# dvl-tum/e-osvos

Measured on AMD Instinct MI355X. Metric: finetune_iters_per_sec, higher is better.
Workload: dtype f32 (f16x3 split); 1 GPU; e-OSVOS-50 fine-tune iteration (BASELINE configs[1]): DeepLabV3+-ResNet50, batch 3, 480x854, BCE, per-neuron-lr SGD; one (sequence, object) per rank; batch=3, height=480, width=854, parallelism=replicas x1

## Files before the change

e-osvos_amd/_ffi.py:

```python
import ctypes
import os

_HERE = os.path.dirname(os.path.abspath(__file__))
LIB_PATH = os.environ.get('EOSVOS_LIB') or os.path.join(_HERE, 'libeosvos.so')

c_float_p = ctypes.c_void_p
_E = ctypes.c_void_p


class View(ctypes.Structure):
    _fields_ = [('p', ctypes.c_void_p), ('ld', ctypes.c_int), ('key', ctypes.c_void_p), ('ldkey', ctypes.c_int)]


class ConvViews(ctypes.Structure):
    _fields_ = ([(n, ctypes.c_int) for n in ('algo', 'B', 'H', 'W', 'Cin', 'Cout', 'k', 'stride', 'dil', 'pad')] +
                [('w_oihw', ctypes.c_void_p), ('scale', ctypes.c_void_p), ('bias', ctypes.c_void_p), ('passes', ctypes.c_int),
                 ('x', View), ('y', View), ('res', View), ('relu', ctypes.c_int), ('y_m8', ctypes.c_void_p),
                 ('g', View), ('gx', View), ('add', View), ('accum', ctypes.c_int), ('mask_c0', ctypes.c_int),
                 ('gx_m8', ctypes.c_void_p), ('dw_oihw', ctypes.c_void_p),
                 ('slot_bits', ctypes.c_uint * 2), ('slot_valid', ctypes.c_int * 2),
                 ('src_slot_bits', ctypes.c_uint * 2), ('src_slot_valid', ctypes.c_int * 2), ('fwd_slices', ctypes.c_int)])


VIEWS_FWD, VIEWS_DGRAD, VIEWS_WGRAD = 1, 2, 4

_SIGNATURES = {
    'eosvos_version': (ctypes.c_char_p, []),
    'eosvos_last_error': (ctypes.c_char_p, []),
    'eosvos_set_matrix_mode': (ctypes.c_int, [ctypes.c_int]),
    'eosvos_get_matrix_mode': (ctypes.c_int, []),
    'eosvos_set_presplit': (ctypes.c_int, [ctypes.c_int]),
    'eosvos_plan_fingerprint': (ctypes.c_int, [_E, ctypes.POINTER(ctypes.c_uint64)]),
    'eosvos_set_engine_matrix_mode': (ctypes.c_int, [_E, ctypes.c_int]),
    'eosvos_get_engine_matrix_mode': (ctypes.c_int, [_E]),
    'eosvos_set_wg_budget': (ctypes.c_int, [_E, ctypes.c_int]),
    'eosvos_set_side_stream': (ctypes.c_int, [_E, ctypes.c_int]),
    'eosvos_num_convs': (ctypes.c_int, [ctypes.c_int]),
    'eosvos_conv_info': (ctypes.c_int, [ctypes.c_int, ctypes.c_int, ctypes.POINTER(ctypes.c_int64)]),
    'eosvos_param_count': (ctypes.c_int64, [ctypes.c_int]),
    'eosvos_lr_count': (ctypes.c_int64, [ctypes.c_int]),
    'eosvos_norm_count': (ctypes.c_int64, [ctypes.c_int]),
    'eosvos_create': (ctypes.c_int, [ctypes.POINTER(_E), ctypes.c_int, ctypes.c_int, ctypes.c_int,
                                     ctypes.c_int, ctypes.c_int, ctypes.c_int, ctypes.c_void_p]),
    'eosvos_create_ex': (ctypes.c_int, [ctypes.POINTER(_E), ctypes.c_int, ctypes.c_int, ctypes.c_int,
                                        ctypes.c_int, ctypes.c_int, ctypes.c_int, ctypes.c_void_p, ctypes.c_int]),
    'eosvos_destroy': (ctypes.c_int, [_E]),
# ... 190 lines not shown
```

e-osvos_amd/csrc/conv_kernels.hip:

```cpp
#include "kernels.h"
#include "conv_tile.h"

#include <stdlib.h>
#include <string.h>

#include <type_traits>
#include <vector>

namespace eosvos {

typedef float f32x16 __attribute__((ext_vector_type(16)));

#define EOSVOS_BK 32
#define EOSVOS_EB 4
#define EOSVOS_EB128 EOSVOS_EB
#define EOSVOS_OCC 2
#define MFMA32(a, b, c) __builtin_amdgcn_mfma_f32_32x32x2f32((a), (b), (c), 0, 0, 0)

#define EOSVOS_BK_DEEP 16
#define EOSVOS_DEEP_TILES 1024
template <int BN, bool KMAJOR, int DEEP = 0>
__global__ __launch_bounds__(256, DEEP ? 3 : EOSVOS_OCC) void conv_igemm_kernel(const ConvArgs p) {
  constexpr int BM = 128, BK = DEEP == 2 ? EOSVOS_BK_DEEP : EOSVOS_BK;
  constexpr int LDA = BK + 4;
// ... 1491 lines not shown
    const int ranges = a.N / NC;
    int chunks = (target + a.nplanes * ranges - 1) / (a.nplanes * ranges);
    const int max_chunks = a.plane_rows / 128 > 0 ? a.plane_rows / 128 : 1;
    chunks = chunks < 1 ? 1 : (chunks > max_chunks ? max_chunks : chunks);
    a.row_chunks = chunks;
    const int groups8 = (a.nplanes * chunks + 7) / 8 * 8;
    hipLaunchKernelGGL((conv1x1_stream_kernel<K, NC>), dim3(groups8 * ranges), dim3(512), lds, s, a);
    return;
  }
  constexpr int total = 256 * (K <= 128 ? EOSVOS_STREAM_OCC : 1);
  const int ranges = a.N / NC;
  const int wgs = total / ranges > 0 ? total / ranges : 1;
  hipLaunchKernelGGL((conv1x1_stream_kernel<K, NC>), dim3(wgs, ranges), dim3(512), lds, s, a);
}


#define STEM_SLOTS 24
#define STEM_PITCH (STEM_SLOTS * 16 + 32)
__global__ __launch_bounds__(512) void stem_fwd_h3_kernel(const float* __restrict__ xpad, const float* __restrict__ w,
                                                          const float* __restrict__ a, const float* __restrict__ bb,
                                                          float* __restrict__ y, int B, int H, int W, int Ho, int Wo,
                                                          const unsigned* __restrict__ amax_x) {
  __shared__ __attribute__((aligned(16))) unsigned char sw_[2 * 64 * STEM_PITCH];
  __shared__ float s_a[64], s_b[64];
  __shared__ unsigned s_red[8];
  const int tid = threadIdx.x, lane = tid & 63, wave = tid >> 6;
  float wv[3][8];
  unsigned wm = 0;
#pragma unroll
  for (int q = 0; q < 3; ++q) {
// ... 739 lines not shown
  }
  const int T = a.KH * a.KW;
  const int bk = a.deep == 2 ? EOSVOS_BK_DEEP : EOSVOS_BK;
  const long ksteps = (long)T * ((a.Kc + bk - 1) / bk);
  const long sk_tiles = tiles - (long)a.dp_q * nwg;
  const bool fixup = a.splitk > 1 || (a.per > 0 && sk_tiles > 0 && (a.per % ksteps != 0 || a.tprefix));
  if (g_plan_log_on)
    plan_log_add(ConvPlanRec{pk, a.kmajor != 0, bn, (int)tiles, (int)ksteps, a.deep, a.dp_q, a.per, nwg, a.splitk, a.tprefix != nullptr,
                             a.torder != nullptr, fixup, conv_wg_budget(a.wg_budget)});
  if (fixup) {
    ProfScope ps(kProfFixup, 0.0, s);
    with_tile(bn, [&](auto BN) { hipLaunchKernelGGL((conv_fixup_kernel<BN()>), dim3((unsigned)sk_tiles, 8), block, 0, s, a); });
  }
}

#define EOSVOS_WG_BKP 32
#define EOSVOS_WG_OCC 2
template <int BMO, int BNI>
__global__ __launch_bounds__(256, EOSVOS_WG_OCC) void wgrad_kernel(const WgradArgs p) {
  constexpr int BKP = EOSVOS_WG_BKP;
  constexpr int LDA = BMO + 4, LDB = BNI + 4;
  constexpr int A_EL = BKP * LDA, B_EL = BKP * LDB, STAGE = A_EL + B_EL;
  __shared__ __attribute__((aligned(16))) float smem[2 * STAGE];

  const int tid = threadIdx.x, lane = tid & 63, wave = tid >> 6;
  const int wm = wave >> 1, wn = wave & 1;
  const int r = lane & 31, h = lane >> 5;

  const int T = p.KH * p.KW;
  const int ct = (p.Cout + BMO - 1) / BMO, it = (p.Cin + BNI - 1) / BNI;
// ... 227 lines not shown
```

e-osvos_amd/csrc/engine.cpp:

```cpp
#include <dlfcn.h>
#include <hip/hip_runtime.h>
#include <math.h>
#include <stdio.h>
#include <stdlib.h>
#include <string.h>

#include <algorithm>
#include <cmath>
#include <functional>
#include <map>
#include <string>
#include <vector>

#include "../../include/eosvos.h"
#include "kernels.h"
#include "scratch_layout.h"
#include "tensor_views.h"

using namespace eosvos;

static thread_local std::string g_err;
static int fail(const std::string& m) {
  g_err = m;
  return 1;
// ... 633 lines not shown
  return m;
}
void wino_ensure_weights(eosvos_engine* e, int ci, int tm, hipStream_t st) {
  auto& w = e->wino[ci];
  if (w.us_valid) return;
  const ConvL& c = e->t.convs[ci];
  unsigned* us = amax_wino_weights(e, ci, st);
  launch_wino_weight(tm, e->W_(ci), c.cout, c.cin, e->A_(ci), w.U, w.Us, st, us, us ? us + e->t.convs.size() : nullptr);
  w.us_valid = true;
}
struct Opt {
  View add_;
  bool relu_ = false, side_ = false, accum_ = false;
  const Tensor* mask_ = nullptr;
  int mask_c0_ = 0;
  Opt& add(const View& v) { add_ = v; return *this; }
  Opt& relu(bool on = true) { relu_ = on; return *this; }
  Opt& side(bool on = true) { side_ = on; return *this; }
  Opt& accum(bool on = true) { accum_ = on; return *this; }
  Opt& mask(const Tensor* x, int c0 = 0) { mask_ = x; mask_c0_ = c0; return *this; }
};
void conv_fwd(eosvos_engine* e, int ci, const View& xv, const View& yv, int B, const Opt& o = Opt()) {
  const float *x = xv.ptr(), *res = o.add_.ptr();
  float* y = yv.ptr();
  const int ldx = xv.ld(), ldy = yv.ld(), ldres = o.add_.ld(), Hi = xv.t->H, Wi = xv.t->W;
  const bool relu = o.relu_, side = o.side_;
  const ConvL& c = e->t.convs[ci];
  ConvArgs a;
  memset(&a, 0, sizeof(a));
  a.wg_budget = e->wg_budget;
  hipStream_t st = side ? e->s2 : e->s;
  const Written yw = twrite_fused(e, yv);
  a.x = x; a.w = e->W_(ci); a.y = y; a.ws = side ? e->ws_conv2 : e->ws_conv;
  a.B = B; a.Hi = Hi; a.Wi = Wi; a.ldx = ldx; a.Kc = c.cin;
  a.Ho = conv_out(Hi, c.k, c.stride, c.dil, c.pad); a.Wo = conv_out(Wi, c.k, c.stride, c.dil, c.pad);
// ... 28 lines not shown
  } else {
    a.scale = e->A_(ci); a.bias = e->B_(ci);
    a.res = res; a.ldres = ldres; a.relu = relu ? 1 : 0;
    if (relu && yw.mask) { a.mask8_out = yw.mask; a.ldm8_out = yw.ldmask; }
  }
  attach_tap_table(e, ci, 0, B, a);
  if (h3_mode() && !amax_init(e)) {
    amax_weights(e, st);
    a.amax_x = tlookup(e, *xv.t);
    if (!a.amax_x) a.amax_x = amax_get(e, AM_X, ci, x, (long)B * Hi * Wi, c.cin, ldx, st);
    a.amax_w = amax_slot(e, AM_W, ci);
    if (!gn) a.amax_y = yw.slot;
  }
  if (!gn && !side) pair_attach(e, yv, a);
  trace("fwd", ci, a.M, a.N, (long)c.T() * c.cin, conv_plan(a), conv_exec_frac(a));
  launch_conv(a, st);
  pair_covered(e, *yv.t, a);
  if (gn)
    launch_gn_forward(e->zbuf[ci]->p, c.cout, e->G_(ci), e->nb + c.noff, res, ldres, y, ldy, e->gn_stats[ci], e->gn_partial, B,
                      a.Ho * a.Wo, c.cout, 1e-5f, relu ? 1 : 0, st, yw.slot, relu ? yw.mask : nullptr, yw.ldmask);
}
bool dgrad_has_tail(const ConvArgs& a) { return a.N > 128 && a.N % 128 > 0 && a.N % 128 <= 64; }
void launch_dgrad_tail_split(eosvos_engine* e, int ci, ConvArgs a, long K) {
  const int tail = a.N % 128;
  ConvArgs b = a;
  a.N -= tail;
  trace("dgrad", ci, a.M, a.N, K, conv_plan(a));
  launch_conv(a, e->s);
  b.N = tail; b.w += a.N; b.y += a.N;
  if (b.mask8) { b.mask8 += a.N / 4; b.mask_c0 = b.mask_c0 > a.N ? b.mask_c0 - a.N : 0; }
// ... 56 lines not shown
    launch_wino_dgrad_output(wg.tm, e->wino_dv, prow, c.cin, B, Hin, Win, th, tw, wg.d, mask8, a.ldm8, a.mask_c0, a.accum, gx, ldgx, e->s, gxs);
    return 0;
  }
  if (c.k == 1 && c.stride == 2 && !add) {
    if (!a.accum) (void)hipMemsetAsync(gx, 0, (size_t)B * Hin * Win * ldgx * sizeof(float), e->s);
    a.Ho = a.Hi; a.Wo = a.Wi; a.mul = 1; a.off0 = 0; a.kstep = 0; a.upshift = 0;
    a.M = B * a.Ho * a.Wo; a.dst_up = 1; a.Hf = Hin; a.Wf = Win;
  }
  if (dgrad_has_tail(a) && !a.dst_up && !(c.k == 3 && c.dil >= 2)) {
    launch_dgrad_tail_split(e, ci, a, (long)c.T() * c.cout);
    return 0;
  }
  attach_tap_table(e, ci, 1, B, a);
  pair_attach(e, gxv, a);
  trace("dgrad", ci, a.M, a.N, (long)c.T() * c.cout, conv_plan(a), conv_exec_frac(a));
  launch_conv(a, e->s);
  pair_covered(e, *gxv.t, a);
  return 0;
}
#define EOSVOS_SIDE_BATCH 4
int wgp_budget(const eosvos_engine* e) {
  constexpr int share = 75;
  int b = conv_wg_budget_of(e->wg_budget);
  if (e->s2) b = conv_clamp_wg_budget(std::max(64, b * share / 100 / 64 * 64));
  return b;
}
int pair_margin(int phase) {
  static const int margin_x = getenv("EOSVOS_TUNE_PAIR_MARGIN_X") ? atoi(getenv("EOSVOS_TUNE_PAIR_MARGIN_X")) : 2;
  static const int margin_g = getenv("EOSVOS_TUNE_PAIR_MARGIN_G") ? atoi(getenv("EOSVOS_TUNE_PAIR_MARGIN_G")) : 3;
  return phase == 0 ? margin_x : margin_g;
}
bool pair_operand(eosvos_engine* e, const View& v, long rows, PairBuf*& pb) {
  const long rows_alloc = e->lastB > 0 ? rows / e->lastB * e->maxB : rows;
// ... 431 lines not shown
  if (mode != EOSVOS_MATRIX_F32 && mode != EOSVOS_MATRIX_BF16X6 && mode != EOSVOS_MATRIX_F16X3) return fail("unknown matrix mode");
  conv_set_mfma_mode(mode);
  return 0;
}
int eosvos_get_matrix_mode(void) { return conv_mfma_mode(); }
int eosvos_plan_fingerprint(eosvos_engine* e, uint64_t* out2) {
  if (!e || !out2) return fail("null argument");
  out2[0] = e->plan_fp[0]; out2[1] = e->plan_fp[1];
  return 0;
}
int eosvos_set_presplit(int on) {
  const int prev = presplit_switch() ? g_presplit : 0;
  g_presplit = on == 2 ? 2 : (on ? 1 : 0);
  return prev;
}
int eosvos_set_engine_matrix_mode(eosvos_engine* e, int mode) {
  if (!e) return fail("null engine");
  if (mode != -1 && mode != EOSVOS_MATRIX_F32 && mode != EOSVOS_MATRIX_BF16X6 && mode != EOSVOS_MATRIX_F16X3) return fail("unknown matrix mode");
  e->mode = mode;
  return 0;
}
int eosvos_get_engine_matrix_mode(eosvos_engine* e) {
  if (!e) { fail("null engine"); return -1; }
  return e->mode >= 0 ? e->mode : conv_mfma_mode();
}
int eosvos_set_wg_budget(eosvos_engine* e, int workgroups) {
  if (!e) { fail("null engine"); return -1; }
  if (workgroups < 0) { fail("workgroup budget must be >= 0"); return -1; }
  const int b = conv_clamp_wg_budget(workgroups);
  if (b == e->wg_budget) return b;
// ... 534 lines not shown
    bool any = false;
    for (int ci = 0; ci < (int)e->wino.size(); ++ci) {
      if (!e->wino[ci].V || e->wino[ci].us_valid || ci >= (int)e->conv_hin.size() || !e->conv_hin[ci]) continue;
      const ConvL& c = t.convs[ci];
      const int Ho = conv_out(e->conv_hin[ci], c.k, c.stride, c.dil, c.pad), Wo = conv_out(e->conv_win[ci], c.k, c.stride, c.dil, c.pad);
      if (!wino_on(e, ci, B, Ho, Wo)) continue;
      if (!any) { fork(0); any = true; }
      wino_ensure_weights(e, ci, wino_geom(e, c, B, Ho, Wo).tm, e->s2);
    }
    if (any) { (void)hipEventRecord(e->ev_wino_w, e->s2); e->wino_w_wait = true; }
  }
  const View dcat_low(e->dcat, 256, 48);
  for (size_t i = 0; i < t.blocks.size(); ++i) {
    const Block& b = t.blocks[i];
    auto& f = e->bb[i];
    if (b.ds >= 0) {
      if (fside) fork(b.ds);
      conv_fwd(e, b.ds, f.xin, f.dsb, B, Opt().side(fside));
      if (fside) (void)hipEventRecord(e->ev[b.c3], e->s2);
    }
    conv_fwd(e, b.c1, f.xin, f.t1, B, Opt().relu());
    conv_fwd(e, b.c2, f.t1, f.t2, B, Opt().relu());
    if (b.ds >= 0 && fside) (void)hipStreamWaitEvent(s, e->ev[b.c3], 0);
    conv_fwd(e, b.c3, f.t2, f.out, B, Opt().relu().add(b.ds >= 0 ? f.dsb : f.xin));
    if ((int)i == t.layer1_last_block && fside && !t.v3) {
      fork(t.dec1);
      conv_fwd(e, t.dec1, f.out, dcat_low, B, Opt().relu().side());
      (void)hipEventRecord(e->ev[t.dec_a], e->s2);
    }
  }
  Tensor* const l4 = e->bb.back().out;
  const int P16 = e->h16 * e->w16;
  hipStream_t ps = fside ? e->s2 : s;
  if (fside) fork(t.pool);
  auto pool_branch = [&]() {
    launch_colsum(l4->p, l4->C, e->vec, B, P16, 2048, 1.0f / (float)P16, e->colscratch, ps);
    if (e->gn()) {
      launch_gemv_fwd(e->W_(t.pool), e->vec, nullptr, nullptr, e->zbuf[t.pool]->p, B, 256, 2048, ps);
      launch_gn_forward(e->zbuf[t.pool]->p, 256, e->G_(t.pool), e->nb + t.convs[t.pool].noff, nullptr, 0, e->poolout, 256,
// ... 126 lines not shown
  for (int i = l4_frozen ? -1 : (int)t.blocks.size() - 1; i >= 0; --i) {
    if (i == first_l4_block - 1) {
      if (flush_part0()) return 1;
      if (frozen) break;
    }
    const Block& b = t.blocks[i];
    auto& f = e->bb[i];
    conv_wgrad(e, b.c3, f.g_out, f.t2, B);
    if (conv_dgrad(e, b.c3, f.g_out, f.g_t2, B, Opt().mask(f.t2))) return 1;
    conv_wgrad(e, b.c2, f.g_t2, f.t1, B);
    if (conv_dgrad(e, b.c2, f.g_t2, f.g_t1, B, Opt().mask(f.t1))) return 1;
    const bool is_first_block = i == 0;
    bool have = !t.v3 && (i == t.layer1_last_block + 1);
    const Tensor* inmask = is_first_block ? nullptr : f.xin;
    const bool in_frozen = frozen && b.c1 == e->train_from;
    if (b.ds >= 0) {
      conv_wgrad(e, b.ds, f.g_out, f.xin, B);
      if (!in_frozen && conv_dgrad(e, b.ds, f.g_out, f.g_xin, B, Opt().accum(have))) return 1;
      conv_wgrad(e, b.c1, f.g_t1, f.xin, B);
      if (!in_frozen && conv_dgrad(e, b.c1, f.g_t1, f.g_xin, B, Opt().accum().mask(inmask))) return 1;
    } else {
      if (have) return fail("internal: identity block after the low-level tap is unsupported");
      conv_wgrad(e, b.c1, f.g_t1, f.xin, B);
      if (conv_dgrad(e, b.c1, f.g_t1, f.g_xin, B, Opt().mask(inmask).add(f.g_out))) return 1;
    }
    if (b.ds >= 0 && flush_wgrad_group(e, t.stage[b.c1], B)) return 1;
  }
  if (!frozen) {
  const auto& xrec = amax_rec_of(e, AM_X, 0);
  const bool stem_h3 = h3_mode() && e->amax && xrec.epoch == e->fwd_epoch && xrec.ptr == e->xpad;
  unsigned* ag = stem_h3 ? amax_fused_slot(e, AM_G, 0, e->gn() ? e->zbuf[0]->p : e->g_c1->p, s) : nullptr;
// ... 1966 lines not shown
```

e-osvos_amd/csrc/kernels.h:

```cpp
#pragma once
#include <hip/hip_runtime.h>
#include <stdint.h>

namespace eosvos {
#define AMAX_SUB 32
#define AMAX_ROW 2048
#if defined(__HIPCC__)
__device__ __forceinline__ unsigned amax_f1(float x) {
  const unsigned a = __float_as_uint(x) & 0x7fffffffu;
  return a < 0x7f800000u ? a : 0u;
}
__device__ __forceinline__ unsigned amax_f4(unsigned m, const float4& v) {
  const unsigned a = amax_f1(v.x), b = amax_f1(v.y), c = amax_f1(v.z), d = amax_f1(v.w);
  const unsigned ab = a > b ? a : b, cd = c > d ? c : d;
  const unsigned q = ab > cd ? ab : cd;
  return m > q ? m : q;
}
__device__ __forceinline__ uint8_t relu_bits(const float4& v) {
  return (uint8_t)((v.x > 0.f ? 1 : 0) | (v.y > 0.f ? 2 : 0) | (v.z > 0.f ? 4 : 0) | (v.w > 0.f ? 8 : 0));
}
__device__ __forceinline__ void relu_mask8(float4& v, unsigned bits) {
  v.x = (bits & 1u) ? v.x : 0.f; v.y = (bits & 2u) ? v.y : 0.f; v.z = (bits & 4u) ? v.z : 0.f; v.w = (bits & 8u) ? v.w : 0.f;
}
template <int WAVES = 4>
// ... 114 lines not shown
#endif
inline int conv_par_pixel(int B, int Ho, int Wo, int m) {
  const int He = (Ho + 1) >> 1, Hod = Ho >> 1, We = (Wo + 1) >> 1, Wod = Wo >> 1;
  const int n00 = B * He * We, n01 = B * He * Wod, n10 = B * Hod * We;
  int py, px, r = m;
  if (r < n00) { py = 0; px = 0; }
  else if ((r -= n00) < n01) { py = 0; px = 1; }
  else if ((r -= n01) < n10) { py = 1; px = 0; }
  else { r -= n10; py = 1; px = 1; }
  const int Hc = py ? Hod : He, Wc = px ? Wod : We;
  const int nc = Hc * Wc;
  const int b = r / nc, rr = r - b * nc;
  const int cy = rr / Wc, cx = rr - cy * Wc;
  return (b * Ho + 2 * cy + py) * Wo + 2 * cx + px;
}
void launch_conv(ConvArgs& a, hipStream_t s);
int conv_bn(const ConvArgs& a);
int conv_plan(ConvArgs& a);
void conv_set_mfma_mode(int mode);
void conv_set_thread_mfma_mode(int mode);
int conv_thread_mfma_mode();
void conv_prof_enable(int on);
int conv_prof_read(int max, const char** names, long* counts, double* ms, double* flops);
void conv_prof_mark_begin(int kernel, double flops, hipStream_t s);
void conv_prof_mark_end(hipStream_t s);
struct ConvPlanRec {
  int kernel;
  int kmajor, bn;
  int tiles, ksteps;
  int deep, dp_q, per, nwg, splitk;
  int tprefix, torder;
// ... 13 lines not shown
  X(kProfConvIgemm_2, "conv_igemm_kernel<64, false, 0>") X(kProfConvIgemm_3, "conv_igemm_kernel<64, true, 0>") \
  X(kProfWgrad, "wgrad_kernel<128, 128>") X(kProfWgrad_1, "wgrad_kernel<128, 64>") \
  X(kProfWgrad_2, "wgrad_kernel<64, 128>") X(kProfWgrad_3, "wgrad_kernel<64, 64>") \
  X(kProfFixup, "conv_fixup_kernel") \
  X(kProfWgradX6Group, "wgrad_x6_group_kernel<128, 128>") X(kProfWgradX6Group_1, "wgrad_x6_group_kernel<128, 64>") \
  X(kProfWgradX6Group_2, "wgrad_x6_group_kernel<64, 128>") X(kProfWgradX6Group_3, "wgrad_x6_group_kernel<64, 64>") \
  X(kProfConvH3, "conv_h3_kernel<128, false>") X(kProfConvH3_1, "conv_h3_kernel<128, true>") \
  X(kProfConvH3_2, "conv_h3_kernel<64, false>") X(kProfConvH3_3, "conv_h3_kernel<64, true>") \
  X(kProfWgradH3, "wgrad_h3_kernel<128, 128>") X(kProfWgradH3_1, "wgrad_h3_kernel<128, 64>") \
  X(kProfWgradH3_2, "wgrad_h3_kernel<64, 128>") X(kProfWgradH3_3, "wgrad_h3_kernel<64, 64>") \
  X(kProfWgradH3Group, "wgrad_h3_group_kernel<128, 128>") X(kProfWgradH3Group_1, "wgrad_h3_group_kernel<128, 64>") \
  X(kProfWgradH3Group_2, "wgrad_h3_group_kernel<64, 128>") X(kProfWgradH3Group_3, "wgrad_h3_group_kernel<64, 64>") \
  X(kProfConvH3Multi, "conv_h3_multi_kernel") X(kProfConvX6Multi, "conv_x6_multi_kernel") \
  X(kProfStream1x1_128, "conv1x1_stream_kernel<*, 128>") X(kProfStream1x1_64, "conv1x1_stream_kernel<*, 64>") \
  X(kProfStream3x3, "conv3x3_stream_kernel") \
  X(kProfWgradP, "wgrad_p_kernel<256, 256>") X(kProfWgradPGroup, "wgrad_p_group_kernel<256, 256>")
enum ProfKernel {
#define EOSVOS_PROF_ID(id, name) id,
  EOSVOS_PROF_KERNELS(EOSVOS_PROF_ID)
#undef EOSVOS_PROF_ID
  kProfKernels
};
double conv_exec_frac(const struct ConvArgs& a);
double wgrad_exec_frac(const struct WgradArgs& a);
int conv_mfma_mode();
void launch_absmax(const float* x, long rows, int C, int ld, unsigned* slot, hipStream_t s);
void launch_amax_zero(unsigned* first, int count, hipStream_t s);
void launch_absmax_segments(const float* base, const long* dev_off, const int* dev_n, int nseg, unsigned* slots, hipStream_t s);
double launch_mfma_probe(float* scratch, int iters, hipStream_t s);
int64_t conv_ws_floats();
}
// ... 295 lines not shown
```

e-osvos_amd/engine.py:

```python
import collections
import ctypes
import functools

import torch

from . import _ffi, bootstrap, boundary, cldice, loss_sum, potts, surface
from .loss_names import LOSS_KINDS, resolve_cap, resolve_loss, resolve_radius
from .topology import ARCH_ID, norm_layers, trainable


def _ptr(t):
    return ctypes.c_void_p(t.data_ptr())


def _optr(t):
    return _ptr(t) if t is not None else None


def _chunks(n, step):
    return ((f, min(f + step, n)) for f in range(0, n, step))


def _keep_flags(keep, n):
    flags = bytearray(n)
# ... 279 lines not shown
    def _check_images(self, images):
        self._check_stream()
        assert images.is_cuda and images.dtype == torch.float32 and images.is_contiguous()
        b, c, h, w = images.shape
        assert c == 3 and h == self.height and w == self.width and 1 <= b <= self.max_batch, images.shape
        return b

    @property
    def matrix_mode(self):
        return _MODE_NAMES[self.lib.eosvos_get_engine_matrix_mode(self.h)]

    def set_engine_matrix_mode(self, mode):
        _ffi.check(self.lib.eosvos_set_engine_matrix_mode(self.h, -1 if mode is None else _MODE_IDS[mode]))
        self._own_mode = mode
        self._guard_fell_back = False

    def plan_fingerprint(self):
        out = (ctypes.c_uint64 * 2)()
        _ffi.check(self.lib.eosvos_plan_fingerprint(self.h, out))
        return int(out[0]), int(out[1])

    def _new_state_for_guard(self):
        if getattr(self, '_guard_fell_back', False):
            self._guard_fell_back = False
            self.set_engine_matrix_mode(None)
        self._verify_pending = True

    def _fall_back(self, reason, diff, scale):
        import warnings
        self.set_engine_matrix_mode('bf16x6')
# ... 1044 lines not shown
```

include/eosvos.h:

```cpp
#ifndef EOSVOS_H
#define EOSVOS_H

#include <stddef.h>
#include <stdint.h>

#ifdef __cplusplus
extern "C" {
#endif

typedef struct eosvos_engine eosvos_engine;

#define EOSVOS_ARCH_RESNET50 50
#define EOSVOS_ARCH_RESNET101 101
#define EOSVOS_ARCH_V3_RESNET50 1050
#define EOSVOS_ARCH_V3_RESNET101 1101
#define EOSVOS_NORM_BN_FROZEN 0
#define EOSVOS_NORM_GN16 1

const char* eosvos_version(void);
const char* eosvos_last_error(void);

#define EOSVOS_MATRIX_F32 0
#define EOSVOS_MATRIX_BF16X6 1
#define EOSVOS_MATRIX_F16X3 2
int eosvos_set_matrix_mode(int mode);
int eosvos_get_matrix_mode(void);
int eosvos_set_presplit(int on);
int eosvos_plan_fingerprint(eosvos_engine* e, uint64_t* out2);
int eosvos_set_engine_matrix_mode(eosvos_engine* e, int mode);
int eosvos_get_engine_matrix_mode(eosvos_engine* e);

int eosvos_set_wg_budget(eosvos_engine* e, int workgroups);

int eosvos_set_side_stream(eosvos_engine* e, int on);

int eosvos_num_convs(int arch);
int eosvos_conv_info(int arch, int idx, int64_t* info);
int64_t eosvos_param_count(int arch);
int64_t eosvos_lr_count(int arch);
int64_t eosvos_norm_count(int arch);

int eosvos_create(eosvos_engine** out, int arch, int norm_mode, int height, int width,
// ... 266 lines not shown
```

Measured before the change: 114.9 finetune_iters/s.

## Fuse bottleneck main and downsample 1x1 convs into one branch-sum kernel

Adds a conv1x1_branch_kernel that computes the bottleneck's last 1x1 conv and its stride-1 downsample 1x1 conv in one launch and sums them in registers. In forward it replaces the side-stream downsample plus the residual-add conv. In backward it replaces the two dgrad launches that accumulate into the same input gradient. The aim is to drop a launch, a round trip of the downsample/intermediate tensor through memory, and a cross-stream event wait. The cost is that it only handles specific K/N shapes in f16x3 mode and gives up the side-stream overlap, and it falls back to the separate convs when the eligibility checks fail.

```diff
diff --git a/e-osvos_amd/_ffi.py b/e-osvos_amd/_ffi.py
--- a/e-osvos_amd/_ffi.py
+++ b/e-osvos_amd/_ffi.py
@@ -30,6 +30,8 @@
     'eosvos_set_matrix_mode': (ctypes.c_int, [ctypes.c_int]),
     'eosvos_get_matrix_mode': (ctypes.c_int, []),
     'eosvos_set_presplit': (ctypes.c_int, [ctypes.c_int]),
+    'eosvos_set_branch_fusion': (ctypes.c_int, [ctypes.c_int]),
+    'eosvos_test_branch_rowmap': (ctypes.c_int, [ctypes.c_int] * 4),
     'eosvos_plan_fingerprint': (ctypes.c_int, [_E, ctypes.POINTER(ctypes.c_uint64)]),
     'eosvos_set_engine_matrix_mode': (ctypes.c_int, [_E, ctypes.c_int]),
     'eosvos_get_engine_matrix_mode': (ctypes.c_int, [_E]),
diff --git a/e-osvos_amd/csrc/conv_kernels.hip b/e-osvos_amd/csrc/conv_kernels.hip
--- a/e-osvos_amd/csrc/conv_kernels.hip
+++ b/e-osvos_amd/csrc/conv_kernels.hip
@@ -1529,6 +1529,207 @@
   hipLaunchKernelGGL((conv1x1_stream_kernel<K, NC>), dim3(wgs, ranges), dim3(512), lds, s, a);
 }
 
+constexpr int br_it(int K, int NC) { return (NC * (K / 8) + 511) / 512; }
+template <int K, int NC, bool KMAJ>
+__device__ __forceinline__ void br_load_w(float (&raw)[br_it(K, NC)][8], const float* __restrict__ w, int wK, int n0, int tid) {
+  constexpr int GR = NC * (K / 8), IT = br_it(K, NC);
+#pragma unroll
+  for (int it = 0; it < IT; ++it) {
+    const int i = tid + it * 512;
+    if (!KMAJ) {
+      const int r = (i < GR ? i : 0) / (K / 8), c8 = i % (K / 8);
+      const float* src = w + (size_t)(n0 + r) * wK + c8 * 8;
+      const float4 lo = ldg4(src), hi = ldg4(src + 4);
+      raw[it][0] = lo.x; raw[it][1] = lo.y; raw[it][2] = lo.z; raw[it][3] = lo.w;
+      raw[it][4] = hi.x; raw[it][5] = hi.y; raw[it][6] = hi.z; raw[it][7] = hi.w;
+    } else {
+      const int c8 = (i < GR ? i : 0) / NC, r = i % NC;
+      const float* src = w + (size_t)(c8 * 8) * wK + n0 + r;
+#pragma unroll
+      for (int j = 0; j < 8; ++j) raw[it][j] = src[(size_t)j * wK];
+    }
+  }
+}
+template <int K, int NC, bool KMAJ>
+__device__ __forceinline__ void br_store_w(const float (&raw)[br_it(K, NC)][8], unsigned char* img, float sw, int tid) {
+  constexpr int GR = NC * (K / 8), IT = br_it(K, NC), PITCH = frag_pitch(K * 2);
+#pragma unroll
+  for (int it = 0; it < IT; ++it) {
+    const int i = tid + it * 512;
+    if (i < GR) {
+      const int r = KMAJ ? i % NC : i / (K / 8), c8 = KMAJ ? i / NC : i % (K / 8);
+      uint4 h0, h1;
+      s1_split8(make_float4(raw[it][0], raw[it][1], raw[it][2], raw[it][3]), make_float4(raw[it][4], raw[it][5], raw[it][6], raw[it][7]), sw, h0, h1);
+      *reinterpret_cast<uint4*>(img + r * PITCH + c8 * 16) = h0;
+      *reinterpret_cast<uint4*>(img + NC * PITCH + r * PITCH + c8 * 16) = h1;
+    }
+  }
+}
+template <int K, int NC, bool TILED>
+__device__ __forceinline__ void br_ksteps(float4 (&xr)[(K + 31) / 32][2], const float* qn, bool more, const float* s_ks, bool kscale, float sx,
+                                          const unsigned char* img, int fr, int fq, f32x4 (&acc)[NC / 16]) {
+  constexpr int KS = (K + 31) / 32, NF = NC / 16, FH = NF < 4 ? NF : 4, PITCH = frag_pitch(K * 2);
+  constexpr bool KTAIL = (K % 32) != 0;
+#pragma unroll
+  for (int ks = 0; ks < KS; ++ks) {
+    float4 a = xr[ks][0], b = xr[ks][1];
+    const bool live = !KTAIL || ks * 32 + fq * 8 < K;
+    if (more && live) {
+      xr[ks][0] = ldg4(qn + ks * 32);
+      xr[ks][1] = ldg4(qn + ks * 32 + 4);
+    }
+    if (kscale) {
+      const float4 k0 = *reinterpret_cast<const float4*>(s_ks + ks * 32 + fq * 8), k1 = *reinterpret_cast<const float4*>(s_ks + ks * 32 + fq * 8 + 4);
+      a.x *= k0.x; a.y *= k0.y; a.z *= k0.z; a.w *= k0.w;
+      b.x *= k1.x; b.y *= k1.y; b.z *= k1.z; b.w *= k1.w;
+    }
+    uint4 x0, x1;
+    s1_split8(a, b, sx, x0, x1);
+    const int koffs = live ? ks * 64 + fq * 16 : 0;
+#pragma unroll
+    for (int h0 = 0; h0 < NF; h0 += FH) {
+      uint4 w0[FH], w1[FH];
+#pragma unroll
+      for (int f = 0; f < FH; ++f) {
+        const unsigned char* wp = img + ((h0 + f) * 16 + fr) * PITCH + koffs;
+        w0[f] = *reinterpret_cast<const uint4*>(wp);
+        w1[f] = *reinterpret_cast<const uint4*>(wp + NC * PITCH);
+      }
+      if (!TILED) {
+#pragma unroll
+        for (int f = 0; f < FH; ++f) acc[h0 + f] = MFMA_F16(__builtin_bit_cast(f16x8, w1[f]), __builtin_bit_cast(f16x8, x0), acc[h0 + f]);
+#pragma unroll
+        for (int f = 0; f < FH; ++f) acc[h0 + f] = MFMA_F16(__builtin_bit_cast(f16x8, w0[f]), __builtin_bit_cast(f16x8, x1), acc[h0 + f]);
+      } else {
+#pragma unroll
+        for (int f = 0; f < FH; ++f) acc[h0 + f] = MFMA_F16(__builtin_bit_cast(f16x8, w0[f]), __builtin_bit_cast(f16x8, x1), acc[h0 + f]);
+#pragma unroll
+        for (int f = 0; f < FH; ++f) acc[h0 + f] = MFMA_F16(__builtin_bit_cast(f16x8, w1[f]), __builtin_bit_cast(f16x8, x0), acc[h0 + f]);
+      }
+#pragma unroll
+      for (int f = 0; f < FH; ++f) acc[h0 + f] = MFMA_F16(__builtin_bit_cast(f16x8, w0[f]), __builtin_bit_cast(f16x8, x0), acc[h0 + f]);
+      __builtin_amdgcn_sched_barrier(0);
+    }
+  }
+}
+template <int K0, int K1, int NC, bool KMAJ, bool T0, bool T1>
+__global__ __launch_bounds__(512, 1) void conv1x1_branch_kernel(const ConvBranchArgs p) {
+#pragma clang fp contract(off)
+  constexpr int WAVES = 8;
+  constexpr int KS0 = (K0 + 31) / 32, KS1 = (K1 + 31) / 32, NF = NC / 16;
+  constexpr int P0 = frag_pitch(K0 * 2), P1 = frag_pitch(K1 * 2);
+  static_assert(NC <= WAVES * 64 && K0 <= WAVES * 64 && K1 <= WAVES * 64 && K0 % 8 == 0 && K1 % 8 == 0, "one factor per thread");
+  extern __shared__ __attribute__((aligned(16))) unsigned char br_smem[];
+  unsigned char* const img0 = br_smem;
+  unsigned char* const img1 = br_smem + 2 * NC * P0;
+  float* const s_sc0 = reinterpret_cast<float*>(img1 + 2 * NC * P1);
+  float* const s_bi0 = s_sc0 + NC;
+  float* const s_sc1 = s_bi0 + NC;
+  float* const s_bi1 = s_sc1 + NC;
+  float* const s_ks0 = s_bi1 + NC;
+  float* const s_ks1 = s_ks0 + KS0 * 32;
+  const int tid = threadIdx.x, lane = tid & 63, wave = tid >> 6;
+  const int n0 = blockIdx.y * NC;
+  const ConvBranchSeg& g0 = p.seg[0];
+  const ConvBranchSeg& g1 = p.seg[1];
+  const float f_sc0 = (!KMAJ && tid < NC) ? g0.scale[n0 + tid] : 1.f, f_bi0 = (!KMAJ && tid < NC) ? g0.bias[n0 + tid] : 0.f;
+  const float f_sc1 = (!KMAJ && tid < NC) ? g1.scale[n0 + tid] : 1.f, f_bi1 = (!KMAJ && tid < NC) ? g1.bias[n0 + tid] : 0.f;
+  const float f_ks0 = (KMAJ && g0.kscale && tid < K0) ? g0.kscale[tid] : 1.f;
+  const float f_ks1 = (KMAJ && g1.kscale && tid < K1) ? g1.kscale[tid] : 1.f;
+  const unsigned ax0 = amax_issue(g0.amax_x), aks0 = amax_issue(KMAJ ? g0.amax_ks : nullptr), aw0 = amax_issue(g0.amax_w);
+  const unsigned ax1 = amax_issue(g1.amax_x), aks1 = amax_issue(KMAJ ? g1.amax_ks : nullptr), aw1 = amax_issue(g1.amax_w);
+  float sx0, sw0, inv0, sx1, sw1, inv1;
+  {
+    float raw0[br_it(K0, NC)][8], raw1[br_it(K1, NC)][8];
+    br_load_w<K0, NC, KMAJ>(raw0, g0.w, g0.wK, n0, tid);
+    br_load_w<K1, NC, KMAJ>(raw1, g1.w, g1.wK, n0, tid);
+    if (tid < NC) { s_sc0[tid] = f_sc0; s_bi0[tid] = f_bi0; s_sc1[tid] = f_sc1; s_bi1[tid] = f_bi1; }
+    if (tid < KS0 * 32) s_ks0[tid] = f_ks0;
+    if (tid < KS1 * 32) s_ks1[tid] = f_ks1;
+    float ix, iw;
+    sx0 = h3_scale_bits(ax0, KMAJ && g0.amax_ks, aks0, ix);
+    sw0 = h3_scale_bits(aw0, false, 0u, iw);
+    inv0 = ix * iw;
+    sx1 = h3_scale_bits(ax1, KMAJ && g1.amax_ks, aks1, ix);
+    sw1 = h3_scale_bits(aw1, false, 0u, iw);
+    inv1 = ix * iw;
+    br_store_w<K0, NC, KMAJ>(raw0, img0, sw0, tid);
+    br_store_w<K1, NC, KMAJ>(raw1, img1, sw1, tid);
+  }
+  __syncthreads();
+  const int fr = lane & 15, fq = lane >> 4;
+  const int nstrips = (p.M + 15) / 16;
+  const int gstride = gridDim.x * WAVES;
+  auto row_of = [&](int strip) { const int m = strip * 16 + fr; return m < p.M ? m : p.M - 1; };
+  auto src1_of = [&](int m) { return p.seg1_fine ? conv_fine_of_coarse(p.Hf, p.Wf, m) : m; };
+  float4 xr0[KS0][2], xr1[KS1][2];
+  int strip = blockIdx.x * WAVES + wave;
+  if (strip < nstrips) {
+    const int m = row_of(strip);
+    const float* q0 = g0.x + (size_t)m * g0.ldx + fq * 8;
+    const float* q1 = g1.x + (size_t)src1_of(m) * g1.ldx + fq * 8;
+#pragma unroll
+    for (int ks = 0; ks < KS0; ++ks) {
+      if (K0 % 32 == 0 || ks * 32 + fq * 8 < K0) { xr0[ks][0] = ldg4(q0 + ks * 32); xr0[ks][1] = ldg4(q0 + ks * 32 + 4); }
+      else xr0[ks][0] = xr0[ks][1] = make_float4(0.f, 0.f, 0.f, 0.f);
+    }
+#pragma unroll
+    for (int ks = 0; ks < KS1; ++ks) {
+      if (K1 % 32 == 0 || ks * 32 + fq * 8 < K1) { xr1[ks][0] = ldg4(q1 + ks * 32); xr1[ks][1] = ldg4(q1 + ks * 32 + 4); }
+      else xr1[ks][0] = xr1[ks][1] = make_float4(0.f, 0.f, 0.f, 0.f);
+    }
+  }
+  unsigned ymax = 0;
+  for (; strip < nstrips; strip += gstride) {
+    const int nxt = strip + gstride;
+    const bool more = nxt < nstrips;
+    const int mn = row_of(more ? nxt : strip);
+    const float* qn0 = g0.x + (size_t)mn * g0.ldx + fq * 8;
+    const float* qn1 = g1.x + (size_t)src1_of(mn) * g1.ldx + fq * 8;
+    const bool ok = strip * 16 + fr < p.M;
+    const size_t row = (size_t)row_of(strip);
+    f32x4 acc0[NF], acc1[NF];
+#pragma unroll
+    for (int f = 0; f < NF; ++f) { acc0[f] = f32x4{0.f, 0.f, 0.f, 0.f}; acc1[f] = f32x4{0.f, 0.f, 0.f, 0.f}; }
+    br_ksteps<K0, NC, T0>(xr0, qn0, more, s_ks0, KMAJ && g0.kscale, sx0, img0, fr, fq, acc0);
+    br_ksteps<K1, NC, T1>(xr1, qn1, more, s_ks1, KMAJ && g1.kscale, sx1, img1, fr, fq, acc1);
+    const int mc = (KMAJ && p.addend) ? conv_coarse_of_fine(p.H, p.W, (int)row) : -1;
+#pragma unroll
+    for (int f = 0; f < NF; ++f) {
+      const int n = n0 + f * 16 + 4 * fq;
+      float v[4];
+      if (!KMAJ) {
+        const float4 s0 = *reinterpret_cast<const float4*>(s_sc0 + (n - n0)), b0 = *reinterpret_cast<const float4*>(s_bi0 + (n - n0));
+        const float4 s1 = *reinterpret_cast<const float4*>(s_sc1 + (n - n0)), b1 = *reinterpret_cast<const float4*>(s_bi1 + (n - n0));
+#pragma unroll
+        for (int j = 0; j < 4; ++j) {
+          const float r = ((acc1[f][j] * inv1) * f4c(s1, j)) + f4c(b1, j);
+          const float c = ((acc0[f][j] * inv0) * f4c(s0, j)) + f4c(b0, j);
+          v[j] = c + r;
+          if (p.relu) v[j] = fmaxf(v[j], 0.f);
+        }
+      } else {
+        float4 t = make_float4(acc1[f][0] * inv1, acc1[f][1] * inv1, acc1[f][2] * inv1, acc1[f][3] * inv1);
+        if (ok) ymax = amax_f4(ymax, t);
+        if (mc >= 0) {
+          const float4 c4 = ldg4(p.addend + (size_t)mc * p.ldadd + n);
+          t = make_float4(c4.x + t.x, c4.y + t.y, c4.z + t.z, c4.w + t.w);
+          if (ok) ymax = amax_f4(ymax, t);
+        }
+#pragma unroll
+        for (int j = 0; j < 4; ++j) v[j] = (acc0[f][j] * inv0) + f4c(t, j);
+      }
+      float4 o = make_float4(v[0], v[1], v[2], v[3]);
+      if (KMAJ && p.mask8) relu_mask8(o, p.mask8[row * p.ldm8 + (n >> 2)]);
+      if (ok) {
+        *reinterpret_cast<float4*>(p.y + row * p.ldy + n) = o;
+        if (p.mask8_out && p.relu) p.mask8_out[row * p.ldm8_out + (n >> 2)] = relu_bits(o);
+        ymax = amax_f4(ymax, o);
+      }
+    }
+  }
+  if (p.amax_y) amax_block_commit<8>(ymax, p.amax_y);
+}
 
 #define STEM_SLOTS 24
 #define STEM_PITCH (STEM_SLOTS * 16 + 32)
@@ -2298,6 +2499,49 @@
   }
 }
 
+int conv_launch_kind(ConvArgs& a) {
+  if (conv_mfma_mode() != 2 || stream3x3_ok(a) || a.nseg > 0) return 0;
+  if (stream1x1_nc(a)) return 1;
+  const int bn = conv_bn(a);
+  const int nwg = conv_plan(a);
+  const long tiles = (long)((a.M + 127) / 128) * ((a.N + bn - 1) / bn);
+  const long ksteps = (long)a.KH * a.KW * ((a.Kc + EOSVOS_BK - 1) / EOSVOS_BK);
+  const long sk_tiles = tiles - (long)a.dp_q * nwg;
+  const bool shared = a.splitk > 0 || (a.per > 0 && sk_tiles > 0 && (a.per % ksteps != 0 || a.tprefix));
+  return (a.deep || shared || a.tprefix) ? 0 : 2;
+}
+template <int K0, int K1, int NC, bool KMAJ, bool T0, bool T1>
+static void launch_branch_as(const ConvBranchArgs& a, hipStream_t s) {
+  constexpr int lds = 2 * NC * (frag_pitch(K0 * 2) + frag_pitch(K1 * 2)) + (4 * NC + (K0 + 31) / 32 * 32 + (K1 + 31) / 32 * 32) * 4;
+  static_assert(lds <= 160 * 1024, "LDS of a workgroup");
+  static bool attr = false;
+  if (!attr) { (void)hipFuncSetAttribute((const void*)conv1x1_branch_kernel<K0, K1, NC, KMAJ, T0, T1>, hipFuncAttributeMaxDynamicSharedMemorySize, lds); attr = true; }
+  const int ranges = a.N / NC;
+  const dim3 grid(256 / ranges > 0 ? 256 / ranges : 1, ranges);
+  hipLaunchKernelGGL((conv1x1_branch_kernel<K0, K1, NC, KMAJ, T0, T1>), grid, dim3(512), lds, s, a);
+}
+template <int K0, int K1, int NC, bool KMAJ>
+static void launch_branch(const ConvBranchArgs& a, hipStream_t s) {
+  const bool t0 = a.seg[0].tiled != 0, t1 = a.seg[1].tiled != 0;
+  if (!t0 && !t1) launch_branch_as<K0, K1, NC, KMAJ, false, false>(a, s);
+  else if (!t0 && t1) launch_branch_as<K0, K1, NC, KMAJ, false, true>(a, s);
+  else if (t0 && t1) launch_branch_as<K0, K1, NC, KMAJ, true, true>(a, s);
+}
+static int branch_nc(int K0, int K1, int N, int kmajor) {
+  if (!kmajor && K0 == 64 && K1 == 64 && N % 128 == 0) return 128;
+  if (kmajor && K0 == 64 && K1 == 256 && N == 64) return 64;
+  return 0;
+}
+bool conv_branch_shape(int K0, int K1, int N, int kmajor) { return branch_nc(K0, K1, N, kmajor) != 0; }
+bool conv_branch_orders(int tiled0, int tiled1) { return !(tiled0 && !tiled1); }
+void launch_conv_branch(const ConvBranchArgs& a, hipStream_t s) {
+  if (g_plan_log_on) { ConvPlanRec r{}; r.kernel = kProfBranch1x1; r.kmajor = a.kmajor; plan_log_add(r); }
+  ProfScope ps(kProfBranch1x1, 2.0 * a.M * a.N * ((double)a.seg[0].K + a.seg[1].K), s);
+  const int K0 = a.seg[0].K, K1 = a.seg[1].K;
+  if (!a.kmajor && K0 == 64 && K1 == 64) launch_branch<64, 64, 128, false>(a, s);
+  else if (a.kmajor && K0 == 64 && K1 == 256) launch_branch<64, 256, 64, true>(a, s);
+}
+
 #define EOSVOS_WG_BKP 32
 #define EOSVOS_WG_OCC 2
 template <int BMO, int BNI>
diff --git a/e-osvos_amd/csrc/engine.cpp b/e-osvos_amd/csrc/engine.cpp
--- a/e-osvos_amd/csrc/engine.cpp
+++ b/e-osvos_amd/csrc/engine.cpp
@@ -671,11 +671,13 @@
   bool relu_ = false, side_ = false, accum_ = false;
   const Tensor* mask_ = nullptr;
   int mask_c0_ = 0;
+  ConvArgs* defer_ = nullptr;
   Opt& add(const View& v) { add_ = v; return *this; }
   Opt& relu(bool on = true) { relu_ = on; return *this; }
   Opt& side(bool on = true) { side_ = on; return *this; }
   Opt& accum(bool on = true) { accum_ = on; return *this; }
   Opt& mask(const Tensor* x, int c0 = 0) { mask_ = x; mask_c0_ = c0; return *this; }
+  Opt& defer(ConvArgs* out) { defer_ = out; return *this; }
 };
 void conv_fwd(eosvos_engine* e, int ci, const View& xv, const View& yv, int B, const Opt& o = Opt()) {
   const float *x = xv.ptr(), *res = o.add_.ptr();
@@ -734,6 +736,7 @@
   }
   if (!gn && !side) pair_attach(e, yv, a);
   trace("fwd", ci, a.M, a.N, (long)c.T() * c.cin, conv_plan(a), conv_exec_frac(a));
+  if (o.defer_) { *o.defer_ = a; return; }
   launch_conv(a, st);
   pair_covered(e, *yv.t, a);
   if (gn)
@@ -820,9 +823,49 @@
   attach_tap_table(e, ci, 1, B, a);
   pair_attach(e, gxv, a);
   trace("dgrad", ci, a.M, a.N, (long)c.T() * c.cout, conv_plan(a), conv_exec_frac(a));
+  if (o.defer_) { *o.defer_ = a; return 0; }
   launch_conv(a, e->s);
   pair_covered(e, *gxv.t, a);
   return 0;
+}
+int g_branch_fusion = 1;
+bool branch_sum_candidate(const eosvos_engine* e, int B, long M, int K0, int K1, int N, int kmajor) {
+  if (!g_branch_fusion || !h3_mode() || e->gn() || e->force_algo != 0 || !e->s2 || e->train_from != 0) return false;
+  const long min_m = g_branch_fusion == 2 ? 1 : (B == 1 ? 1024 : 16384);
+  return M >= min_m && conv_branch_shape(K0, K1, N, kmajor);
+}
+ConvBranchSeg branch_seg(const ConvArgs& a, int kind) {
+  ConvBranchSeg g;
+  g.x = a.x; g.ldx = a.ldx; g.w = a.w; g.wK = a.wK; g.K = a.Kc;
+  g.scale = a.scale; g.bias = a.bias; g.kscale = a.kscale;
+  g.amax_x = a.amax_x; g.amax_w = a.amax_w; g.amax_ks = a.amax_ks;
+  g.tiled = kind == 2 ? 1 : 0;
+  return g;
+}
+bool launch_branch_sum(eosvos_engine* e, int ci_main, ConvArgs& main, int ci_side, ConvArgs& side) {
+  const int km = main.kmajor;
+  const int k0 = conv_launch_kind(main), k1 = conv_launch_kind(side);
+  if (!k0 || !k1 || !conv_branch_orders(k0 == 2, k1 == 2)) return false;
+  if (side.kmajor != km || main.M != side.M || main.N != side.N || main.y2 || side.y2) return false;
+  if (main.KH != 1 || side.KH != 1 || main.dst_up || side.dst_up || main.upshift || side.upshift || main.mul != 1 || side.mul != 1) return false;
+  if ((main.ldx & 3) || (side.ldx & 3) || (main.ldy & 3) || !main.amax_x || !side.amax_x || !main.amax_w || !side.amax_w) return false;
+  if (!conv_branch_shape(main.Kc, side.Kc, main.N, km)) return false;
+  if (!km) {
+    if (main.res != side.y || main.ldres != side.ldy || !main.relu || side.relu || side.res || main.accum || side.accum) return false;
+    if (!main.scale || !main.bias || !side.scale || !side.bias || main.mask8 || side.mask8) return false;
+  } else {
+    if (main.y != side.y || main.ldy != side.ldy || !main.accum || side.accum || main.res || side.res || side.mask8) return false;
+    if (main.mask8 || main.amax_y != side.amax_y) return false;
+  }
+  ConvBranchArgs p;
+  memset(&p, 0, sizeof(p));
+  p.seg[0] = branch_seg(main, k0); p.seg[1] = branch_seg(side, k1);
+  p.y = main.y; p.ldy = main.ldy; p.M = main.M; p.N = main.N; p.H = main.Ho; p.W = main.Wo; p.kmajor = km;
+  p.relu = main.relu; p.mask8_out = main.mask8_out; p.ldm8_out = main.ldm8_out;
+  p.amax_y = main.amax_y;
+  if (trace_on()) fprintf(stderr, "EOSVOS_BRANCH main=%d side=%d\n", ci_main, ci_side);
+  launch_conv_branch(p, e->s);
+  return true;
 }
 #define EOSVOS_SIDE_BATCH 4
 int wgp_budget(const eosvos_engine* e) {
@@ -1284,6 +1327,14 @@
   g_presplit = on == 2 ? 2 : (on ? 1 : 0);
   return prev;
 }
+int eosvos_set_branch_fusion(int on) {
+  const int prev = g_branch_fusion;
+  g_branch_fusion = on == 2 ? 2 : (on ? 1 : 0);
+  return prev;
+}
+int eosvos_test_branch_rowmap(int dir, int H, int W, int m) {
+  return dir ? conv_coarse_of_fine(H, W, m) : conv_fine_of_coarse(H, W, m);
+}
 int eosvos_set_engine_matrix_mode(eosvos_engine* e, int mode) {
   if (!e) return fail("null engine");
   if (mode != -1 && mode != EOSVOS_MATRIX_F32 && mode != EOSVOS_MATRIX_BF16X6 && mode != EOSVOS_MATRIX_F16X3) return fail("unknown matrix mode");
@@ -1848,15 +1899,29 @@
   for (size_t i = 0; i < t.blocks.size(); ++i) {
     const Block& b = t.blocks[i];
     auto& f = e->bb[i];
-    if (b.ds >= 0) {
+    ConvArgs a_ds, a_c3;
+    const bool sum = b.ds >= 0 && fside && t.convs[b.ds].stride == 1 &&
+                     branch_sum_candidate(e, B, (long)B * f.out->H * f.out->W, t.convs[b.c3].cin, t.convs[b.ds].cin, t.convs[b.c3].cout, 0);
+    if (sum) {
+      conv_fwd(e, b.ds, f.xin, f.dsb, B, Opt().defer(&a_ds));
+    } else if (b.ds >= 0) {
       if (fside) fork(b.ds);
       conv_fwd(e, b.ds, f.xin, f.dsb, B, Opt().side(fside));
       if (fside) (void)hipEventRecord(e->ev[b.c3], e->s2);
     }
     conv_fwd(e, b.c1, f.xin, f.t1, B, Opt().relu());
     conv_fwd(e, b.c2, f.t1, f.t2, B, Opt().relu());
-    if (b.ds >= 0 && fside) (void)hipStreamWaitEvent(s, e->ev[b.c3], 0);
-    conv_fwd(e, b.c3, f.t2, f.out, B, Opt().relu().add(b.ds >= 0 ? f.dsb : f.xin));
+    if (sum) {
+      conv_fwd(e, b.c3, f.t2, f.out, B, Opt().relu().add(f.dsb).defer(&a_c3));
+      if (!launch_branch_sum(e, b.c3, a_c3, b.ds, a_ds)) {
+        launch_conv(a_ds, s);
+        launch_conv(a_c3, s);
+        pair_covered(e, *f.out, a_c3);
+      }
+    } else {
+      if (b.ds >= 0 && fside) (void)hipStreamWaitEvent(s, e->ev[b.c3], 0);
+      conv_fwd(e, b.c3, f.t2, f.out, B, Opt().relu().add(b.ds >= 0 ? f.dsb : f.xin));
+    }
     if ((int)i == t.layer1_last_block && fside && !t.v3) {
       fork(t.dec1);
       conv_fwd(e, t.dec1, f.out, dcat_low, B, Opt().relu().side());
@@ -2013,7 +2078,21 @@
     bool have = !t.v3 && (i == t.layer1_last_block + 1);
     const Tensor* inmask = is_first_block ? nullptr : f.xin;
     const bool in_frozen = frozen && b.c1 == e->train_from;
-    if (b.ds >= 0) {
+    const bool sum = b.ds >= 0 && !in_frozen && !have && !inmask && t.convs[b.ds].stride == 1 &&
+                     branch_sum_candidate(e, B, (long)B * f.g_xin->H * f.g_xin->W, t.convs[b.c1].cout, t.convs[b.ds].cout, t.convs[b.c1].cin, 1);
+    if (sum) {
+      ConvArgs a_ds, a_c1;
+      conv_wgrad(e, b.ds, f.g_out, f.xin, B);
+      if (conv_dgrad(e, b.ds, f.g_out, f.g_xin, B, Opt().defer(&a_ds))) return 1;
+      conv_wgrad(e, b.c1, f.g_t1, f.xin, B);
+      if (conv_dgrad(e, b.c1, f.g_t1, f.g_xin, B, Opt().accum().defer(&a_c1))) return 1;
+      if (!launch_branch_sum(e, b.c1, a_c1, b.ds, a_ds)) {
+        launch_conv(a_ds, e->s);
+        pair_covered(e, *f.g_xin, a_ds);
+        launch_conv(a_c1, e->s);
+        pair_covered(e, *f.g_xin, a_c1);
+      }
+    } else if (b.ds >= 0) {
       conv_wgrad(e, b.ds, f.g_out, f.xin, B);
       if (!in_frozen && conv_dgrad(e, b.ds, f.g_out, f.g_xin, B, Opt().accum(have))) return 1;
       conv_wgrad(e, b.c1, f.g_t1, f.xin, B);
diff --git a/e-osvos_amd/csrc/kernels.h b/e-osvos_amd/csrc/kernels.h
--- a/e-osvos_amd/csrc/kernels.h
+++ b/e-osvos_amd/csrc/kernels.h
@@ -152,7 +152,53 @@
   const int cy = rr / Wc, cx = rr - cy * Wc;
   return (b * Ho + 2 * cy + py) * Wo + 2 * cx + px;
 }
+#if defined(__HIPCC__)
+__host__ __device__
+#endif
+inline int conv_fine_of_coarse(int H, int W, int mc) {
+  const int Hc = (H + 1) >> 1, Wc = (W + 1) >> 1;
+  const int b = mc / (Hc * Wc), rem = mc - b * (Hc * Wc);
+  const int cy = rem / Wc, cx = rem - cy * Wc;
+  return (b * H + 2 * cy) * W + 2 * cx;
+}
+#if defined(__HIPCC__)
+__host__ __device__
+#endif
+inline int conv_coarse_of_fine(int H, int W, int mf) {
+  const int Hc = (H + 1) >> 1, Wc = (W + 1) >> 1;
+  const int b = mf / (H * W), rem = mf - b * (H * W);
+  const int y = rem / W, x = rem - y * W;
+  if ((y | x) & 1) return -1;
+  return (b * Hc + (y >> 1)) * Wc + (x >> 1);
+}
 void launch_conv(ConvArgs& a, hipStream_t s);
+int conv_launch_kind(ConvArgs& a);
+struct ConvBranchSeg {
+  const float* x; int ldx;
+  const float* w; int wK;
+  int K;
+  const float* scale; const float* bias;
+  const float* kscale;
+  const unsigned* amax_x; const unsigned* amax_w; const unsigned* amax_ks;
+  int tiled;
+};
+struct ConvBranchArgs {
+  ConvBranchSeg seg[2];
+  float* y; int ldy;
+  int M, N;
+  int H, W;
+  int kmajor;
+  int seg1_fine;
+  int Hf, Wf;
+  const float* addend; int ldadd;
+  int relu;
+  uint8_t* mask8_out; int ldm8_out;
+  const uint8_t* mask8; int ldm8;
+  unsigned* amax_y;
+};
+bool conv_branch_shape(int K0, int K1, int N, int kmajor);
+bool conv_branch_orders(int tiled0, int tiled1);
+void launch_conv_branch(const ConvBranchArgs& a, hipStream_t s);
 int conv_bn(const ConvArgs& a);
 int conv_plan(ConvArgs& a);
 void conv_set_mfma_mode(int mode);
@@ -196,7 +242,8 @@
   X(kProfConvH3Multi, "conv_h3_multi_kernel") X(kProfConvX6Multi, "conv_x6_multi_kernel") \
   X(kProfStream1x1_128, "conv1x1_stream_kernel<*, 128>") X(kProfStream1x1_64, "conv1x1_stream_kernel<*, 64>") \
   X(kProfStream3x3, "conv3x3_stream_kernel") \
-  X(kProfWgradP, "wgrad_p_kernel<256, 256>") X(kProfWgradPGroup, "wgrad_p_group_kernel<256, 256>")
+  X(kProfWgradP, "wgrad_p_kernel<256, 256>") X(kProfWgradPGroup, "wgrad_p_group_kernel<256, 256>")       \
+  X(kProfBranch1x1, "conv1x1_branch_kernel")
 enum ProfKernel {
 #define EOSVOS_PROF_ID(id, name) id,
   EOSVOS_PROF_KERNELS(EOSVOS_PROF_ID)
diff --git a/e-osvos_amd/engine.py b/e-osvos_amd/engine.py
--- a/e-osvos_amd/engine.py
+++ b/e-osvos_amd/engine.py
@@ -317,6 +317,9 @@
         _ffi.check(self.lib.eosvos_set_engine_matrix_mode(self.h, -1 if mode is None else _MODE_IDS[mode]))
         self._own_mode = mode
         self._guard_fell_back = False
+
+    def set_branch_fusion(self, on):
+        return int(self.lib.eosvos_set_branch_fusion(int(on)))
 
     def plan_fingerprint(self):
         out = (ctypes.c_uint64 * 2)()
diff --git a/include/eosvos.h b/include/eosvos.h
--- a/include/eosvos.h
+++ b/include/eosvos.h
@@ -26,6 +26,8 @@
 int eosvos_set_matrix_mode(int mode);
 int eosvos_get_matrix_mode(void);
 int eosvos_set_presplit(int on);
+int eosvos_set_branch_fusion(int on);
+int eosvos_test_branch_rowmap(int dir, int H, int W, int m);
 int eosvos_plan_fingerprint(eosvos_engine* e, uint64_t* out2);
 int eosvos_set_engine_matrix_mode(eosvos_engine* e, int mode);
 int eosvos_get_engine_matrix_mode(eosvos_engine* e);
```

After: 115.8 finetune_iters/s, median of 6. No clear change (+0.8%).
